# Charrrrrlie/X-as-Supervision

Measured on AMD Instinct MI355X. Metric: images/sec HM36_Multi_SurS1 256px bs32 (full disc+gen training step), higher is better.
Workload: dtype f32 (f16x3 split: every fp32 operand as two fp16 pieces, three products; f32 accumulate); 1 GPU; HM36_Multi_SurS1; batch_per_gpu=32, cameras=4, image=256x256, parallelism=dp1, ranks=1, precision=f16x3, dedupe=False, full=False

## Files before the change

include/xas_hip.h:

```cpp
#ifndef XAS_HIP_H
#define XAS_HIP_H

#include <stddef.h>
#include <stdint.h>

#ifdef __cplusplus
extern "C" {
#endif

const char* xas_last_error(void);
enum {
  XAS_TUNE_WGRAD_SPLIT_XCD = 1,
  XAS_TUNE_PLAIN_KLOOP = 32,
  XAS_TUNE_GLOBAL_LOAD = 64,
  XAS_TUNE_WGRAD_GLOBAL_LOAD = 128,
  XAS_TUNE_WGRAD_ALT_ORDER = 8192,
  XAS_TUNE_WGRAD_PLAIN_KLOOP = 524288,
  XAS_TUNE_SLAB_SHIFT = 15,
  XAS_TUNE_SLAB_MASK = 3,
  XAS_TUNE_SLAB_512 = 32768,
  XAS_TUNE_SLAB_128 = 65536,
  XAS_TUNE_SLAB_64 = 98304,
  XAS_TUNE_COL_REDUCE_LEAN = 262144,
  XAS_TUNE_GENERAL_KERNELS = 1 << 22,
  XAS_TUNE_NO_WIDE_TILES = 1 << 23,
  XAS_TUNE_NO_STEM_WGRAD = 1 << 24,
  XAS_TUNE_STEM_FWD_F32 = 1 << 25,
  XAS_TUNE_NO_X6P = 1 << 26,
  XAS_TUNE_X6P_ANY_K = 1 << 27
};
int xas_set_tuning(int flags);
enum { XAS_PREC_F32 = 0, XAS_PREC_BF16 = 1, XAS_PREC_BF16X6 = 2, XAS_PREC_F16X3 = 3 };
#define XAS_AMAX_SUB 32
#define XAS_AMAX_STRIDE 32
#define XAS_AMAX_SLOT_FLOATS (XAS_AMAX_SUB * XAS_AMAX_STRIDE)
enum { XAS_GRAD_IS_X = 0x100 };
int xas_set_precision(int mode);
int xas_get_precision(void);
int xas_abi_version(void);

#define XAS_HEAD_STATS 16
size_t xas_head_workspace_floats(int B, int K, int D);
int xas_head_softargmax_fwd(const float* logits, int B, int K, int D, int num_hypo, int neighbor,
                            float* kps, int64_t* z_idx, float* depth_prob_map, int groups, float* stats,
                            float* partial, void* stream);
int xas_head_softargmax_from_partials(const float* partial, int B, int K, int D, int nchunk, int num_hypo, int neighbor,
                                      float* kps, int64_t* z_idx, float* depth_prob_map, int groups, float* stats,
                                      void* stream);
int xas_head_softargmax_flip_from_partials(const float* partial, int B, int K, int D, int nchunk, int num_hypo, int neighbor,
                                           const int* perm, float* kps, int64_t* z_idx, float* depth_prob_map, int groups,
                                           void* stream);
int xas_head_softargmax_fwd_flip(const float* logits, int B, int K, int D, int num_hypo, int neighbor, const int* perm,
                                 float* kps, int64_t* z_idx, float* depth_prob_map, int groups, float* partial, void* stream);

int xas_head_softargmax_bwd(const float* logits, const float* stats, const int64_t* z_idx,
                            const float* grad_kps, int B, int K, int D, int num_hypo, int neighbor,
                            float* grad_logits, float* coef, void* stream);
int xas_head_softargmax_bwd_amax(const float* logits, const float* stats, const int64_t* z_idx,
                                 const float* grad_kps, int B, int K, int D, int num_hypo, int neighbor,
                                 float* grad_logits, float* coef, float* amax_out, void* stream);

#define XAS_HEAD_SPREAD 5
size_t xas_head_spread_workspace_floats(int B, int K, int D);
int xas_head_spread(const float* logits, int B, int K, int D, float* spread , float* workspace, void* stream);

#define XAS_GEO_NORM 1
#define XAS_GEO_MONO 2
#define XAS_GEO_PATCH 4
#define XAS_GEO_IMAGE 8
int xas_patch_to_world_fwd(const float* kps, const float* trans_image, const float* k_mat,
                           const float* pelvis, const float* rot_world, const float* trans_world,
                           int B, int Hy, int K, float image_size, float rect_width, int flags,
                           float* world, void* stream);
int xas_patch_to_world_bwd(const float* kps, const float* grad_world, const float* trans_image,
                           const float* k_mat, const float* pelvis, const float* rot_world,
                           const float* trans_world, int B, int Hy, int K, float image_size,
                           float rect_width, int flags, float* grad_kps, void* stream);

#define XAS_GEO_WORLD 16
int xas_world_to_patch_fwd(const float* pts, const float* pre_rot, float pre_scale, int pelvis_origin,
                           const float* trans_image, const float* k_mat, const float* pelvis,
                           const float* rot_world, const float* trans_world, int B, int Hy, int K,
                           float image_size, float rect_width, int flags, float* out, void* stream);
int xas_world_to_patch_bwd(const float* pts, const float* grad_out, const float* pre_rot, float pre_scale,
                           int pelvis_origin, const float* trans_image, const float* k_mat, const float* pelvis,
                           const float* rot_world, const float* trans_world, int B, int Hy, int K,
                           float image_size, float rect_width, int flags, float* grad_pts, float* grad_pre_rot,
                           void* stream);

int xas_lines_nblk(int S);
int xas_draw_lines_max_fwd(const float* kps, long kp_stride_b, long kp_stride_j, int B, int K,
                           const int* parents, const int* children, int L, unsigned fine_mask,
                           float body_width, int S, float* mask, void* stream);
int xas_draw_lines_max_bwd(const float* kps, long kp_stride_b, long kp_stride_j, int B, int K,
                           const int* parents, const int* children, int L, unsigned fine_mask,
                           float body_width, int S, const float* grad_mask, float* partial,
                           float* grad_kps_xy , void* stream);

typedef struct {
  int N, Hi, Wi, Cin;
  int Cout, R, S;
  int stride, pad;
  int Ho, Wo;
  int mode;
  const float* grad_amax;
  const float* x_amax;
} xas_conv_shape;

int xas_conv_weight_planes(const xas_conv_shape* s, int pass);
int xas_conv_kernel_class(const xas_conv_shape* s, int pass);
int xas_f16_weight_overflow(int reset);
int xas_f16_weight_overflow_peek(unsigned* device_out, void* stream);
size_t xas_split_weight_bytes(long rows, long K, int pieces);
// ... 313 lines not shown
```

x-as-supervision_amd/csrc/head.hip:

```cpp
#include "common.h"

namespace xas {

struct HeadGeom {
  int B, K, D, HW, W, C4, G, rec;
  int KT, ntile, C4t;
  int R, rh, rw, wshift;
  int P, nchunk;
};

static int pow2_slots(long C4) {
  int gcd = 1;
  while (gcd < 64 && (C4 % (gcd * 2)) == 0) gcd *= 2;
  return 64 / gcd;
}

static bool pow2_policy(int D, int K) {
  if (!(D >= 4 && D <= 64 && (D & (D - 1)) == 0) || (tune_flags() & XAS_TUNE_GENERAL_KERNELS)) return false;
  if (K <= 0) return true;
  const long C4 = (long)K * (D / 4);
  const int R = pow2_slots(C4);
  return R <= D * D && C4 * R <= 1024;
}

// ... 240 lines not shown
  const float X = a.SX / S, Y = a.SY / S;
  float* st = stats + ((size_t)b * g.K + k) * XAS_HEAD_STATS;
  if (lane == 0) { st[0] = a.M + __logf(S); st[1] = X; st[2] = Y; }
  finalize_tail(g, b, k, pz0, pz1, X, Y, num_hypo, neighbor, kps, z_idx, depth_prob_map, dmap_every, st);
}

__global__ void head_finalize_flip_kernel(const float* __restrict__ partial, HeadGeom g, const int* __restrict__ perm,
                                          int num_hypo, int neighbor, float* __restrict__ kps, int64_t* __restrict__ z_idx,
                                          float* __restrict__ depth_prob_map, int dmap_every) {
  const int b = blockIdx.x / g.K, k = blockIdx.x % g.K;
  const int lane = threadIdx.x;
  const int d0 = lane, d1 = lane + 64;
  const bool live0 = d0 < g.D, live1 = d1 < g.D;
  int k2 = perm[k];
  if ((unsigned)k2 >= (unsigned)g.K) k2 = k;
  const size_t image = (size_t)g.nchunk * g.K * g.rec;
  const ChunkSums a = merge_chunks(partial + b * image + (size_t)k * g.rec, g, d0, d1, live0, live1);
  const ChunkSums m = merge_chunks(partial + ((size_t)(g.B / 2) + b) * image + (size_t)k2 * g.rec, g, d0, d1, live0, live1);
  const float S1 = wave_sum(a.sd0 + a.sd1), S2 = wave_sum(m.sd0 + m.sd1);
  const float pz0 = live0 ? 0.5f * (a.sd0 / S1 + m.sd0 / S2) : 0.f, pz1 = live1 ? 0.5f * (a.sd1 / S1 + m.sd1 / S2) : 0.f;
  const float X = 0.5f * (a.SX / S1 + ((float)(g.W - 1) - m.SX / S2)), Y = 0.5f * (a.SY / S1 + m.SY / S2);
  finalize_tail(g, b, k, pz0, pz1, X, Y, num_hypo, neighbor, kps, z_idx, depth_prob_map, dmap_every, nullptr);
}

__global__ void head_bwd_coef_kernel(const float* __restrict__ stats, const int64_t* __restrict__ z_idx,
                                     const float* __restrict__ grad_kps, HeadGeom g, int num_hypo, int neighbor,
                                     float* __restrict__ coef) {
  const int b = blockIdx.x / g.K, k = blockIdx.x % g.K;
  const int d = threadIdx.x;
  const float* st = stats + ((size_t)b * g.K + k) * XAS_HEAD_STATS;
  const float fD = (float)g.D;
  float gx = 0.f, gy = 0.f, gz = 0.f, c0 = 0.f;
  const int r = neighbor / 2;
  for (int h = 0; h < num_hypo; ++h) {
    const float* gk = grad_kps + (((size_t)b * num_hypo + h) * g.K + k) * 3;
    gx += gk[0];
    gy += gk[1];
    if (neighbor == 0) {
      const float cz = gk[2] * (2.f / fD);
      gz += cz * (float)d;
      c0 -= cz * st[3];
    } else {
      const int idx = (int)z_idx[((size_t)b * g.K + k) * num_hypo + h];
      if (d >= idx - r && d <= idx + r) gz += gk[2] * (2.f / fD) * ((float)d - st[3 + h]) / st[9 + h];
    }
  }
  const float cx = gx * (2.f / fD), cy = gy * (2.f / fD);
  c0 += -cx * st[1] - cy * st[2];
  float* o = coef + ((size_t)b * g.K + k) * (4 + g.D);
  if (d == 0) { o[0] = cx; o[1] = cy; o[2] = c0; o[3] = st[0]; }
  if (d < g.D) o[4 + d] = gz;
}

template <bool POW2>
__global__ void head_bwd_kernel(const float4* __restrict__ logits, const float* __restrict__ coef, HeadGeom g,
                                float4* __restrict__ grad, float* __restrict__ amax_out) {
  __shared__ unsigned s_amax;
  if (threadIdx.x == 0) s_amax = 0u;
  if (amax_out) __syncthreads();
  float amx = 0.f;
  const int KT = POW2 ? g.K : g.KT, C4t = POW2 ? g.C4 : g.C4t;
  const int tid = threadIdx.x;
  const int c4t = tid % C4t, slot = tid / C4t;
  const int kt = c4t / g.G, dq = c4t % g.G;
  const int bz = POW2 ? 0 : blockIdx.z;
  const int k = bz * KT + kt;
  const int b = blockIdx.y, chunk = blockIdx.x;
  const int pix0 = chunk * g.P;
  const int pend = min(g.P, g.HW - pix0);
  if (POW2 || k < g.K) {
    const float* cf = coef + ((size_t)b * g.K + k) * (4 + g.D);
    const float cx = cf[0], cy = cf[1], c0 = cf[2], lse = cf[3];
    const float4 gz = *reinterpret_cast<const float4*>(cf + 4 + 4 * dq);
    const size_t off = ((size_t)b * g.HW + pix0) * g.C4 + (k * g.G + dq);
    PixelWalk<POW2> walk(g, pix0 + slot);
#pragma unroll 4
    for (int p = slot; p < pend; p += g.R) {
      const float4 v = stream_load(logits + off + (size_t)p * g.C4);
      float fh, fw;
      walk.next(g, pix0 + p, &fh, &fw);
      const float lin = cx * fw + cy * fh + c0;
      float4 o;
      o.x = __expf(v.x - lse) * (lin + gz.x);
      o.y = __expf(v.y - lse) * (lin + gz.y);
      o.z = __expf(v.z - lse) * (lin + gz.z);
      o.w = __expf(v.w - lse) * (lin + gz.w);
      amx = amax4(amx, o);
      stream_store(grad + off + (size_t)p * g.C4, o);
    }
  }
  if (amax_out) {
    if (amx > 0.f) atomicMax(&s_amax, __float_as_uint(amx));
    __syncthreads();
    const unsigned sub = (blockIdx.x + (blockIdx.y + bz * gridDim.y) * gridDim.x) % (unsigned)kAmaxSub;
    if (threadIdx.x == 0 && s_amax) atomicMax(reinterpret_cast<unsigned*>(amax_out + sub * kAmaxStride), s_amax);
  }
}

struct SpreadRec { float m, S, uw, uh, Mw, Mh, C; };
constexpr int kSpreadRec = 7;

__device__ __forceinline__ SpreadRec spread_merge(const SpreadRec& a, const SpreadRec& b) {
  SpreadRec r;
  r.m = fmaxf(a.m, b.m);
  const float sa = (a.m == -INFINITY) ? 0.f : __expf(a.m - r.m), sb = (b.m == -INFINITY) ? 0.f : __expf(b.m - r.m);
  const float Sa = a.S * sa, Sb = b.S * sb;
  r.S = Sa + Sb;
  const float f = (r.S == 0.f) ? 0.f : Sb / r.S;
  const float x = Sa * f, dw = b.uw - a.uw, dh = b.uh - a.uh;
  r.uw = a.uw + dw * f;
  r.uh = a.uh + dh * f;
  r.Mw = a.Mw * sa + b.Mw * sb + dw * dw * x;
  r.Mh = a.Mh * sa + b.Mh * sb + dh * dh * x;
  r.C = a.C * sa + b.C * sb + dw * dh * x;
  return r;
}

__device__ __forceinline__ void spread_add(SpreadRec& r, float es, float fw, float fh) {
  const float Sn = r.S + es;
  const float f = (Sn == 0.f) ? 0.f : __fdividef(es, Sn);
  const float x = r.S * f, dw = fw - r.uw, dh = fh - r.uh;
  r.S = Sn;
  r.uw += dw * f;
  r.uh += dh * f;
  r.Mw += dw * dw * x;
  r.Mh += dh * dh * x;
  r.C += dw * dh * x;
}

__device__ __forceinline__ void spread_rescale(SpreadRec& r, float mn) {
  const float sc = __expf(r.m - mn);
  r.m = mn;
  r.S *= sc; r.Mw *= sc; r.Mh *= sc; r.C *= sc;
}

__device__ __forceinline__ SpreadRec spread_read(const float* p) { return {p[0], p[1], p[2], p[3], p[4], p[5], p[6]}; }
__device__ __forceinline__ void spread_write(float* p, const SpreadRec& r) {
  p[0] = r.m; p[1] = r.S; p[2] = r.uw; p[3] = r.uh; p[4] = r.Mw; p[5] = r.Mh; p[6] = r.C;
}

template <bool POW2>
// ... 181 lines not shown
                                                      float* depth_prob_map, int groups, void* stream) {
  XAS_REQUIRE(B > 0 && B <= (1 << 29), "head flip from partials: need 0 < B, got B=%d (the records hold 2B images)", B);
  HeadGeom g;
  if (make_geom(2 * B, K, D, pow2_policy(D, K), &g)) return 1;
  XAS_REQUIRE(partial && perm && kps && depth_prob_map && nchunk >= 1, "head flip from partials: null buffer");
  if (check_modes("head flip from partials", D, num_hypo, neighbor, z_idx, B, groups)) return 1;
  g.nchunk = nchunk;
  return launch_finalize_flip(partial, g, perm, num_hypo, neighbor, kps, z_idx, depth_prob_map, groups, stream);
}

extern "C" int xas_head_softargmax_fwd_flip(const float* logits, int B, int K, int D, int num_hypo, int neighbor, const int* perm,
                                            float* kps, int64_t* z_idx, float* depth_prob_map, int groups, float* partial,
                                            void* stream) {
  XAS_REQUIRE(B > 0 && B <= (1 << 29), "head fwd flip: need 0 < B, got B=%d (the logits hold 2B images)", B);
  const bool pow2 = pow2_policy(D, K);
  HeadGeom g;
  if (make_geom(2 * B, K, D, pow2, &g)) return 1;
  XAS_REQUIRE(logits && perm && kps && depth_prob_map && partial, "head fwd flip: null buffer");
  if (check_modes("head fwd flip", D, num_hypo, neighbor, z_idx, B, groups)) return 1;
  if (launch_partial(logits, partial, g, pow2, "head fwd flip", stream)) return 1;
  return launch_finalize_flip(partial, g, perm, num_hypo, neighbor, kps, z_idx, depth_prob_map, groups, stream);
}

extern "C" size_t xas_head_spread_workspace_floats(int B, int K, int D) {
  HeadGeom g;
  if (make_geom(B, K, D, pow2_policy(D, K), &g)) return 0;
  return (size_t)B * g.nchunk * K * kSpreadRec;
}

extern "C" int xas_head_spread(const float* logits, int B, int K, int D, float* spread, float* workspace, void* stream) {
  const bool pow2 = pow2_policy(D, K);
  HeadGeom g;
  if (make_geom(B, K, D, pow2, &g)) return 1;
  XAS_REQUIRE(logits && spread && workspace, "head spread: null buffer");
  XAS_REQUIRE(((uintptr_t)logits & 15) == 0, "head spread: logits must be 16-byte aligned");
  const size_t lds = spread_lds_bytes(g, pow2);
  XAS_REQUIRE(lds <= 64 * 1024, "head spread: LDS %zu too large", lds);
  XAS_REQUIRE((long)B * K < (1L << 31), "head spread: B=%d K=%d exceed the launch grid", B, K);
  if (check_grid("head spread", g)) return 1;
  hipLaunchKernelGGL(pow2 ? head_spread_partial_kernel<true> : head_spread_partial_kernel<false>, dim3(g.nchunk, g.B, g.ntile),
                     dim3(g.C4t * g.R), lds, as_stream(stream), reinterpret_cast<const float4*>(logits), workspace, g);
  XAS_LAUNCH_CHECK();
  hipLaunchKernelGGL(head_spread_finalize_kernel, dim3(B * K), dim3(64), 0, as_stream(stream), workspace, g, spread);
  XAS_LAUNCH_CHECK();
  return 0;
}

extern "C" int xas_head_softargmax_bwd(const float* logits, const float* stats, const int64_t* z_idx,
                                       const float* grad_kps, int B, int K, int D, int num_hypo, int neighbor,
                                       float* grad_logits, float* coef, void* stream) {
  return xas_head_softargmax_bwd_amax(logits, stats, z_idx, grad_kps, B, K, D, num_hypo, neighbor, grad_logits, coef, nullptr, stream);
}

extern "C" int xas_head_softargmax_bwd_amax(const float* logits, const float* stats, const int64_t* z_idx,
                                            const float* grad_kps, int B, int K, int D, int num_hypo, int neighbor,
                                            float* grad_logits, float* coef, float* amax_out, void* stream) {
  const bool pow2 = pow2_policy(D, K);
  HeadGeom g;
  if (make_geom(B, K, D, pow2, &g)) return 1;
  XAS_REQUIRE(logits && stats && grad_kps && grad_logits && coef, "head bwd: null buffer");
  XAS_REQUIRE(num_hypo >= 1 && num_hypo <= 6, "head bwd: num_hypo %d not in [1,6]", num_hypo);
  XAS_REQUIRE(neighbor == 0 || z_idx != nullptr, "head bwd: z_idx required");
  XAS_REQUIRE((((uintptr_t)logits | (uintptr_t)grad_logits | (uintptr_t)coef) & 15) == 0, "head bwd: 16-byte alignment");
  if (check_grid("head bwd", g)) return 1;
  hipLaunchKernelGGL(head_bwd_coef_kernel, dim3(B * K), dim3(D <= 64 ? 64 : 128), 0, as_stream(stream), stats, z_idx,
                     grad_kps, g, num_hypo, neighbor, coef);
  XAS_LAUNCH_CHECK();
  hipLaunchKernelGGL(pow2 ? head_bwd_kernel<true> : head_bwd_kernel<false>, dim3(g.nchunk, B, g.ntile), dim3(g.C4t * g.R), 0,
                     as_stream(stream), reinterpret_cast<const float4*>(logits), coef, g, reinterpret_cast<float4*>(grad_logits),
                     amax_out);
  XAS_LAUNCH_CHECK();
  return 0;
}
```

x-as-supervision_amd/xas_amd/_lib.py:

```python
import ctypes
import os

import torch

_HERE = os.path.dirname(os.path.abspath(__file__))
LIB_PATH = os.environ.get('XAS_HIP_LIB') or os.path.join(_HERE, 'libxas_hip.so')
_lib = None
ABI_VERSION = 3

_T = {'p': ctypes.c_void_p, 'i': ctypes.c_int, 'l': ctypes.c_long, 'f': ctypes.c_float, 'u': ctypes.c_uint,
      'd': ctypes.c_double, 'z': ctypes.c_size_t}


class ConvShape(ctypes.Structure):
    _fields_ = [(n, ctypes.c_int) for n in ('N', 'Hi', 'Wi', 'Cin', 'Cout', 'R', 'S', 'stride', 'pad', 'Ho', 'Wo', 'mode')] + [
        ('grad_amax', ctypes.c_void_p),
        ('x_amax', ctypes.c_void_p)]


PREC_F32, PREC_BF16, PREC_BF16X6, PREC_F16X3 = 0, 1, 2, 3
PREC_NAMES = {'f32': PREC_F32, 'bf16': PREC_BF16, 'bf16x6': PREC_BF16X6, 'f16x3': PREC_F16X3}

GUARD_FLOATS = 8
GUARD_NORM, GUARD_SCALE, GUARD_SKIP, GUARD_T, GUARD_SKIPPED, GUARD_STEP_SIZE, GUARD_INV_SQRT_BC2, GUARD_NONFINITE = range(8)

TUNE_WGRAD_SPLIT_XCD = 1
TUNE_PLAIN_KLOOP, TUNE_GLOBAL_LOAD, TUNE_WGRAD_GLOBAL_LOAD = 32, 64, 128
TUNE_WGRAD_ALT_ORDER, TUNE_WGRAD_PLAIN_KLOOP = 8192, 524288
TUNE_SLAB_SHIFT, TUNE_SLAB_MASK = 15, 3
TUNE_SLAB_512, TUNE_SLAB_128, TUNE_SLAB_64 = 32768, 65536, 98304
TUNE_COL_REDUCE_LEAN = 262144
TUNE_GENERAL_KERNELS = 1 << 22
TUNE_NO_WIDE_TILES, TUNE_NO_STEM_WGRAD, TUNE_STEM_FWD_F32 = 1 << 23, 1 << 24, 1 << 25
TUNE_NO_X6P, TUNE_X6P_ANY_K = 1 << 26, 1 << 27

PLAN_FIELDS = ('route', 'kernel', 'bm', 'bn', 'pipelined', 'phases', 'pieces', 'patch_width', 'tpb', 'images')
PLAN_ROUTES = (None, 'stem_f16', 'stem_f32', 'thin_vec_to_scalar', 'thin_scalar_to_vec', 'direct', 'mfma')
PLAN_KERNELS = (None, 'igemm_buf', 'igemm', 'igemm_x6', 'igemm_x6t', 'igemm_x6p')


def conv_igemm_plan(shp, pass_, has_bias=False):
    out = (ctypes.c_int * len(PLAN_FIELDS))()
    rc = fn('xas_conv_igemm_plan')(shp, pass_, int(has_bias), ctypes.cast(out, ctypes.c_void_p))
    if rc != 0:
        raise RuntimeError('xas_conv_igemm_plan failed (%d): %s' % (rc, load().xas_last_error().decode()))
    plan = dict(zip(PLAN_FIELDS, out))
    plan['route'], plan['kernel'] = PLAN_ROUTES[plan['route']], PLAN_KERNELS[plan['kernel']]
    return plan


SIGNATURES = {
    'xas_abi_version': ('', 'i'),
    'xas_set_tuning': ('i', 'i'),
    'xas_set_precision': ('i', 'i'),
    'xas_get_precision': ('', 'i'),
    'xas_conv_weight_planes': ('si', 'i'),
    'xas_conv_kernel_class': ('si', 'i'),
    'xas_f16_weight_overflow': ('i', 'i'),
    'xas_f16_weight_overflow_peek': ('pp', 'i'),
    'xas_split_weight_bytes': ('lli', 'z'),
    'xas_split_weight': ('ppllip', 'i'),
    'xas_prepare_weights': ('pilp', 'i'),
    'xas_head_workspace_floats': ('iii', 'z'),
    'xas_head_softargmax_fwd': ('piiiiipppippp', 'i'),
    'xas_head_softargmax_bwd': ('ppppiiiiippp', 'i'),
    'xas_head_softargmax_bwd_amax': ('ppppiiiiipppp', 'i'),
    'xas_patch_to_world_fwd': ('ppppppiiiffipp', 'i'),
    'xas_patch_to_world_bwd': ('pppppppiiiffipp', 'i'),
    'xas_world_to_patch_fwd': ('ppfipppppiiiffipp', 'i'),
    'xas_world_to_patch_bwd': ('pppfipppppiiiffippp', 'i'),
    'xas_lines_nblk': ('i', 'i'),
    'xas_draw_lines_max_fwd': ('plliippiufipp', 'i'),
    'xas_draw_lines_max_bwd': ('plliippiufipppp', 'i'),
    'xas_conv_fwd': ('ppppsp', 'i'),
    'xas_conv_fwd_head_chunks': ('sii', 'i'),
    'xas_conv_fwd_head': ('ppppsiipp', 'i'),
    'xas_head_softargmax_from_partials': ('piiiiiipppipp', 'i'),
    'xas_head_softargmax_flip_from_partials': ('piiiiiippppip', 'i'),
    'xas_head_softargmax_fwd_flip': ('piiiiippppipp', 'i'),
    'xas_head_spread_workspace_floats': ('iii', 'z'),
    'xas_head_spread': ('piiippp', 'i'),
    'xas_conv_fwd_bnstats_workspace_floats': ('si', 'z'),
    'xas_conv_fwd_bnstats': ('pppsippplppppfp', 'i'),
    'xas_conv_dgrad_bn_bwd_workspace_floats': ('si', 'z'),
    'xas_conv_dgrad_bn_bwd': ('ppspppppfidppppppp', 'i'),
    'xas_conv_dgrad': ('pppsp', 'i'),
    'xas_conv_dgrad_acc': ('pppsp', 'i'),
    'xas_conv_dgrad_acc_masked': ('pppsppp', 'i'),
    'xas_conv_igemm_plan': ('siip', 'i'),
    'xas_conv_wgrad_workspace_floats': ('s', 'z'),
    'xas_conv_wgrad': ('ppppsp', 'i'),
    'xas_conv_wgrad_oihw': ('ppppsp', 'i'),
    'xas_conv_wgrad_acc': ('ppppsp', 'i'),
    'xas_pack_weight': ('ppiiiiip', 'i'),
    'xas_unpack_weight': ('ppiiiiip', 'i'),
    'xas_bn_workspace_floats': ('lii', 'z'),
    'xas_bn_stats': ('pliipplppppflp', 'i'),
    'xas_bn_stats_from_partials': ('pliilppplppppfp', 'i'),
    'xas_bn_bwd_sums_from_partials': ('pliippppp', 'i'),
    'xas_bn_sync_merge': ('piiilppppfp', 'i'),
    'xas_col_sum': ('plippp', 'i'),
    'xas_col_sum_acc': ('plippp', 'i'),
    'xas_bn_apply': ('ppppppfiliippp', 'i'),
    'xas_bn_apply_amax': ('ppppppfiliipppp', 'i'),
    'xas_abs_max': ('plpp', 'i'),
    'xas_bn_update_running': ('ppppfliip', 'i'),
    'xas_bn_bwd_reduce': ('pppppppfiliipppppp', 'i'),
    'xas_bn_bwd_apply': ('ppppppppfiliidpppp', 'i'),
    'xas_bn_bwd_apply_amax': ('ppppppppfiliidppppp', 'i'),
    'xas_bn_apply_dual_amax': ('pppppf' 'pppppf' 'lii' 'pppp', 'i'),
    'xas_bn_bwd_reduce_dual': ('ppppppf' 'ppf' 'lii' 'ppp' 'pppp' 'p', 'i'),
    'xas_bn_bwd_apply_dual_amax': ('pppp' 'ppppf' 'ppppf' 'liidd' 'pppp' 'p', 'i'),
    'xas_maxpool3x3s2_fwd': ('piiiippp', 'i'),
    'xas_maxpool3x3s2_bwd': ('ppiiiipp', 'i'),
    'xas_upsample2x_fwd': ('piiiipp', 'i'),
    'xas_upsample2x_bwd': ('piiiipp', 'i'),
    'xas_sigmoid_fwd': ('plpp', 'i'),
    'xas_sigmoid_bwd': ('pplpp', 'i'),
    'xas_nchw_to_nhwc': ('piiiipp', 'i'),
# ... 66 lines not shown
        raise RuntimeError('libxas_hip.so is missing (%s): run `python __graft_entry__.py` to build the HIP '
                           'library; the MI355X path has no CPU fallback' % LIB_PATH)
    lib = ctypes.CDLL(LIB_PATH)
    lib.xas_abi_version.restype = ctypes.c_int
    lib.xas_abi_version.argtypes = []
    if lib.xas_abi_version() != ABI_VERSION:
        raise RuntimeError('%s speaks ABI version %d, this binding expects %d (include/xas_hip.h): rebuild it with '
                           '`python __graft_entry__.py`' % (LIB_PATH, lib.xas_abi_version(), ABI_VERSION))
    lib.xas_last_error.restype = ctypes.c_char_p
    lib.xas_last_error.argtypes = []
    _lib = lib
    mode = os.environ.get('XAS_PRECISION', '')
    if mode != '':
        lib.xas_set_precision.argtypes = [ctypes.c_int]
        lib.xas_set_precision.restype = ctypes.c_int
        if lib.xas_set_precision(int(mode)) != 0:
            raise RuntimeError('XAS_PRECISION=%s: %s' % (mode, lib.xas_last_error().decode()))
    global PREC_DEFAULT
    lib.xas_get_precision.restype = ctypes.c_int
    PREC_DEFAULT = int(lib.xas_get_precision())
    return lib


PREC_DEFAULT = None


_bound = {}


def fn(name):
    f = _bound.get(name)
    if f is None:
        args, ret = SIGNATURES[name]
        f = getattr(load(), name)
        f.argtypes = [ctypes.POINTER(ConvShape) if c == 's' else _T[c] for c in args]
        f.restype = _T[ret]
        _bound[name] = f
    return f


def ptr(t):
    if t is None:
        return None
    if not t.is_cuda:
        raise RuntimeError('xas_amd ops run on the GPU only (got a %s tensor); there is no CPU fallback' % t.device)
    return t.data_ptr()


def stream():
    return torch.cuda.current_stream().cuda_stream


profiler = None


def call(name, *args):
    if profiler is not None and name in profiler.names:
        return profiler.timed_call(name, args)
    rc = fn(name)(*args, stream())
    if rc != 0:
        raise RuntimeError('%s failed (%d): %s' % (name, rc, load().xas_last_error().decode()))


def query(name, *args):
    return fn(name)(*args)
```

x-as-supervision_amd/xas_amd/ops_head.py:

```python
import torch

from . import _lib
from ._lib import call, ptr, query

HEAD_STATS = 16
peak_probe = None
GEO_NORM, GEO_MONO, GEO_PATCH = 1, 2, 4
GEO_IMAGE, GEO_WORLD = 8, 16


def _nhwc_storage(logits):
    if logits.dim() != 4:
        raise RuntimeError('logits must be [B, K*D, H, W]')
    if not logits.is_contiguous(memory_format=torch.channels_last):
        logits = logits.contiguous(memory_format=torch.channels_last)
    return logits


def check_patch_size(x, depth_dim, who):
    if x.dim() != 4 or x.shape[-1] != x.shape[-2] or x.shape[-1] != 4 * depth_dim:
        raise RuntimeError('%s(depth_dim=%d) takes square input patches of side 4 * depth_dim = %d, got input %s: build the '
                           'detector with depth_dim = patch size / 4 (a multiple of 4, at most 128: patches up to 512)'
                           % (who, depth_dim, 4 * depth_dim, tuple(x.shape)))


class _SoftArgmax(torch.autograd.Function):
    @staticmethod
    def forward(ctx, logits, num_kp, num_hypo, neighbor, groups):
        from . import ops_nn
        logits_in = logits
        logits_tail = _nhwc_storage(logits)
        logits = ops_nn._full(logits_tail)
        B, C, H, W = logits.shape
        D = C // num_kp
        if not (C == num_kp * D and D == H == W):
            raise RuntimeError('soft-argmax head needs a heat-map cube D == H == W with D a multiple of 4 in [4,128] '
                               '(got C=%d K=%d H=%d W=%d)' % (C, num_kp, H, W))
        dev = logits.device
        kps = torch.empty(B, num_hypo, num_kp, 3, device=dev, dtype=torch.float32)
        z_idx = torch.empty(B, num_kp, num_hypo, device=dev, dtype=torch.int64)
        dmap = torch.empty(groups, num_kp, D, device=dev, dtype=torch.float32)
        stats = torch.empty(B, num_kp, HEAD_STATS, device=dev, dtype=torch.float32)
        pre = getattr(logits_in, '_xas_head', None)
        if pre is not None and pre[2] == logits_in._version and pre[0].shape[0] == B and pre[0].shape[2] == num_kp:
            ops_nn.head_stats['fused'] += 1
            call('xas_head_softargmax_from_partials', ptr(pre[0]), B, num_kp, D, pre[1], num_hypo, neighbor, ptr(kps), ptr(z_idx),
                 ptr(dmap), groups, ptr(stats))
        else:
            ops_nn.head_stats['separate'] += 1
            ws = torch.empty(query('xas_head_workspace_floats', B, num_kp, D), device=dev, dtype=torch.float32)
            call('xas_head_softargmax_fwd', ptr(logits), B, num_kp, D, num_hypo, neighbor, ptr(kps), ptr(z_idx),
                 ptr(dmap), groups, ptr(stats), ptr(ws))
        if peak_probe is not None:
            peak_probe(z_idx.clone())
        s = B - logits_tail.shape[0]
        kps_prefix = kps[:s] if s else kps[:0]
        kps, z_idx_all = (kps[s:], z_idx) if s else (kps, z_idx)
        ctx.save_for_backward(logits_tail, stats[s:] if s else stats, z_idx[s:] if s else z_idx)
        ctx.cfg = (num_kp, D, num_hypo, neighbor)
        ctx.mark_non_differentiable(z_idx_all, dmap, kps_prefix)
        return kps, dmap, z_idx_all, kps_prefix

    @staticmethod
    def backward(ctx, g_kps, _g_dmap, _g_idx, _g_prefix=None):
        logits, stats, z_idx = ctx.saved_tensors
        K, D, Hy, nb = ctx.cfg
        B = logits.shape[0]
        g_kps = g_kps.contiguous()
        grad = torch.empty_like(logits)
        coef = torch.empty(B * K * (4 + D), device=logits.device, dtype=torch.float32)
        from . import ops_nn
        slot = ops_nn.grad_amax_slot(logits.device)
        call('xas_head_softargmax_bwd_amax', ptr(logits), ptr(stats), ptr(z_idx), ptr(g_kps), B, K, D, Hy, nb,
             ptr(grad), ptr(coef), ptr(slot))
        if slot is not None:
            ops_nn.tag_grad_amax(grad, slot)
        return grad, None, None, None, None


def softargmax_multi(logits, num_kp, num_hypo, neighbor_size, groups=1):
    kps, dmap, idx, prefix = _SoftArgmax.apply(logits, num_kp, num_hypo, neighbor_size, groups)
    _last_prefix[0] = prefix
    return kps, (dmap[0] if groups == 1 else dmap), idx


_last_prefix = [None]


def softargmax_single(logits, num_kp, groups=1):
    kps, dmap, _, prefix = _SoftArgmax.apply(logits, num_kp, 1, 0, groups)
    _last_prefix[0] = prefix
    return kps, (dmap[0] if groups == 1 else dmap)


def flip_perm(flip_pairs, num_kp, device):
    perm = list(range(num_kp))
    for pair in flip_pairs:
        a, b = (int(v) for v in pair)
        if not (0 <= a < num_kp and 0 <= b < num_kp) or a == b:
            raise RuntimeError('flip pair (%d, %d) does not name two of the %d joints' % (a, b, num_kp))
        if perm[a] != a or perm[b] != b:
            raise RuntimeError('flip pair (%d, %d): a joint has two partners' % (a, b))
        perm[a], perm[b] = b, a
    t = torch.tensor(perm, dtype=torch.int32, device=device)
    t._xas_perm_k = num_kp
    return t


def softargmax_flip(heatmap_2b, num_kp, num_hypo, neighbor_size, perm, groups=1):
    from . import ops_nn
    if torch.is_grad_enabled() and heatmap_2b.requires_grad:
        raise RuntimeError('softargmax_flip is an inference path without a backward: call it under torch.no_grad()')
    if ops_nn._prefix[0]:
        raise RuntimeError('softargmax_flip does not run inside a prefix pass')
    logits = _nhwc_storage(heatmap_2b)
    B2, C, H, W = logits.shape
    D = C // num_kp
    if not (C == num_kp * D and D == H == W):
        raise RuntimeError('soft-argmax head needs a heat-map cube D == H == W with D a multiple of 4 in [4,128] '
                           '(got C=%d K=%d H=%d W=%d)' % (C, num_kp, H, W))
    if B2 < 2 or B2 % 2:
        raise RuntimeError('softargmax_flip takes the logits of B images followed by their B mirrors, got %d images' % B2)
    B = B2 // 2
    dev = logits.device
    if not isinstance(perm, torch.Tensor):
        perm = torch.as_tensor(perm)
    if getattr(perm, '_xas_perm_k', None) != num_kp:
        host = perm.detach().cpu().reshape(-1).tolist()
        if len(host) != num_kp or any(int(v) != v or not 0 <= v < num_kp for v in host):
            raise RuntimeError('softargmax_flip: perm must hold %d joint indices in [0, %d), got %s' % (num_kp, num_kp, host))
        perm = perm.to(device=dev, dtype=torch.int32).contiguous()
        perm._xas_perm_k = num_kp
    if perm.device != dev or perm.dtype != torch.int32 or not perm.is_contiguous():
        raise RuntimeError('softargmax_flip: perm must be a contiguous int32 tensor on %s' % dev)
    kps = torch.empty(B, num_hypo, num_kp, 3, device=dev, dtype=torch.float32)
    z_idx = torch.zeros(B, num_kp, num_hypo, device=dev, dtype=torch.int64)
    dmap = torch.empty(groups, num_kp, D, device=dev, dtype=torch.float32)
    pre = getattr(heatmap_2b, '_xas_head', None)
    if pre is not None and pre[2] == heatmap_2b._version and pre[0].shape[0] == B2 and pre[0].shape[2] == num_kp:
        ops_nn.head_stats['fused'] += 1
        call('xas_head_softargmax_flip_from_partials', ptr(pre[0]), B, num_kp, D, pre[1], num_hypo, neighbor_size, ptr(perm),
             ptr(kps), ptr(z_idx), ptr(dmap), groups)
    else:
# ... 191 lines not shown
```

x-as-supervision_amd/xas_amd/ops_nn.py:

```python
import os

import torch
import torch.distributed as dist

from . import _lib
from . import streams
from ._lib import ConvShape, call, ptr, query

CL = torch.channels_last
_weights_epoch = [0]

_groups = [1]

_prefix = [0, 0]


class bn_groups:
    def __init__(self, groups, prefix_groups=0, images_per_group=0):
        self.groups = int(groups)
        self.prefix = [int(prefix_groups) * int(images_per_group), int(prefix_groups)]
        if self.prefix[1] and not (0 < self.prefix[1] < self.groups and images_per_group > 0):
            raise RuntimeError('bn_groups: the no-grad prefix must be a proper, non-empty subset of the groups')

    def __enter__(self):
        self.prev, _groups[0] = _groups[0], self.groups
        self.prev_prefix = list(_prefix)
        _prefix[0], _prefix[1] = self.prefix
        return self

    def __exit__(self, *exc):
        _groups[0] = self.prev
        _prefix[0], _prefix[1] = self.prev_prefix
        if not _prefix[0]:
            _prefix_storages.clear()


_prefix_storages = set()


def mark_prefix_buffer(buf):
    _prefix_storages.add(buf.untyped_storage().data_ptr())


def _full(x):
    s = _prefix[0]
    if not s or x is None:
        return x
    per = x.stride(0)
    off = x.storage_offset() - s * per
    if (x.dim() != 4 or not x.is_contiguous(memory_format=CL) or off < 0
            or (x.storage_offset() + x.numel()) * 4 > x.untyped_storage().nbytes()
            or x.untyped_storage().data_ptr() not in _prefix_storages):
        raise RuntimeError('prefix pass: an activation arrived without its %d prefix images in front of it' % s)
# ... 328 lines not shown
        box = getattr(w, '_xas_epoch', _weights_epoch)
        key = (w.data_ptr(), w._version, box[0])
        if key != self.key:
            self.key, self.packed = key, {}

    def get(self, w, transposed, shp=None, planes=None):
        self._fresh(w)
        if planes is None:
            planes = query('xas_conv_weight_planes', shp, int(transposed)) if shp is not None else 0
        k = (transposed, planes)
        if k in self.packed:
            return self.packed[k]
        if (transposed, 0) not in self.packed:
            co, ci, r, s = w.shape
            if not transposed and r == 1 and s == 1 and w.is_contiguous() and w.data_ptr() % 16 == 0:
                self.packed[(transposed, 0)] = w.detach().view(-1)
            else:
                p = torch.empty(w.numel(), device=w.device, dtype=torch.float32)
                call('xas_pack_weight', ptr(w.detach().contiguous()), ptr(p), co, ci, r, s, int(transposed))
                self.packed[(transposed, 0)] = p
        if planes:
            src = self.packed[(transposed, 0)]
            rows = w.shape[1] if transposed else w.shape[0]
            kk = src.numel() // rows
            sp = torch.empty(query('xas_split_weight_bytes', rows, kk, planes), device=w.device, dtype=torch.uint8)
            call('xas_split_weight', ptr(src), ptr(sp), rows, kk, planes)
            self.packed[k] = sp
        return self.packed[k]


def _col_sum(t2d_ptr_tensor, M, C):
    out = torch.empty(C, device=t2d_ptr_tensor.device, dtype=torch.float32)
    ws = torch.empty(query('xas_bn_workspace_floats', M, C, 1), device=out.device, dtype=torch.float32)
    call('xas_col_sum', ptr(t2d_ptr_tensor), M, C, ptr(out), ptr(ws))
    return out


def _bias_grad(dy, M, C):
    if C % 4 == 0:
        return _col_sum(dy, M, C)
    return dy.reshape(M, C).sum(0)


def _wgrad(x, dy, shp, w_shape, transposed=False):
    co, ci, r, s = shp.Cout, shp.Cin, shp.R, shp.S
    ws = torch.empty(max(1, query('xas_conv_wgrad_workspace_floats', shp)), device=x.device, dtype=torch.float32)
    dw = torch.empty(w_shape, device=x.device, dtype=torch.float32)
    call('xas_conv_wgrad_oihw', ptr(x), ptr(dy), ptr(dw), ptr(ws), shp)
    return dw


HEAD_IN_EPILOGUE = os.environ.get('XAS_HEAD_IN_EPILOGUE', '1') == '1'
head_stats = {'fused': 0, 'separate': 0}


class _Conv2d(torch.autograd.Function):
    @staticmethod
    def forward(ctx, x, weight, bias, stride, pad, cache, head_kd=None):
        x = to_cl(x)
        n, ci, hi, wi = x.shape
        co, ci2, r, s = weight.shape
        if ci != ci2:
            raise RuntimeError('conv2d: input has %d channels, weight expects %d' % (ci, ci2))
        ho, wo = (hi + 2 * pad - r) // stride + 1, (wi + 2 * pad - s) // stride + 1
        shp, x_slot = with_act_amax(_shape(n, hi, wi, ci, co, r, s, stride, pad, ho, wo), x)
        xf = _full(x)
        yf = empty_cl(xf.shape[0], co, ho, wo, x)
        shp_f = _with_n(shp, xf.shape[0])
        chunks = query('xas_conv_fwd_head_chunks', shp_f, head_kd[0], head_kd[1]) if (head_kd and HEAD_IN_EPILOGUE and x.is_cuda) else 0
        if chunks:
            rec = torch.empty(xf.shape[0], chunks, head_kd[0], 3 + head_kd[1], device=x.device, dtype=torch.float32)
            call('xas_conv_fwd_head', ptr(xf), ptr(cache.get(weight, 0, shp_f)), ptr(bias), ptr(yf), shp_f, head_kd[0], head_kd[1], ptr(rec))
        else:
            call('xas_conv_fwd', ptr(xf), ptr(cache.get(weight, 0, shp_f)), ptr(bias), ptr(yf), shp_f)
        y = _tail(yf)
        if chunks:
            y._xas_head = (rec, chunks, y._version)
        ctx.save_for_backward(x, weight, *([bias] if bias is not None else []))
        ctx.shp, ctx.cache, ctx.has_bias, ctx.x_slot = shp, cache, bias is not None, x_slot
        if ctx.needs_input_grad[1]:
            note_use(weight)
        if bias is not None and ctx.needs_input_grad[2]:
            note_use(bias)
        return y

    @staticmethod
    def backward(ctx, dy):
        x, weight, *rest = ctx.saved_tensors
        shp = with_grad_amax(ctx.shp, dy, ctx.x_slot)
        dy = to_cl(dy)
        dx = dw = db = None
        if ctx.needs_input_grad[0]:
            dx = torch.empty_like(x)
            call('xas_conv_dgrad', ptr(dy), ptr(ctx.cache.get(weight, 1, shp)), ptr(dx), shp)
        if ctx.needs_input_grad[1] and not _wgrad_into_grad(x, dy, shp, weight):
            dw = _wgrad(x, dy, shp, weight.shape)
        if ctx.has_bias and ctx.needs_input_grad[2]:
            M = shp.N * shp.Ho * shp.Wo
            if not _bias_into_grad(dy, M, shp.Cout, rest[0]):
                db = _bias_grad(dy, M, shp.Cout)
        return dx, dw, db, None, None, None, None


def conv2d(x, weight, bias, stride, pad, cache, head_kd=None):
    return _Conv2d.apply(x, weight, bias, stride, pad, cache, head_kd)


def _conv_forward(x, weight, stride, pad, cache):
    n, ci, hi, wi = x.shape
    co, ci2, r, s = weight.shape
    if ci != ci2:
        raise RuntimeError('conv2d: input has %d channels, weight expects %d' % (ci, ci2))
    ho, wo = (hi + 2 * pad - r) // stride + 1, (wi + 2 * pad - s) // stride + 1
    shp, _ = with_act_amax(_shape(n, hi, wi, ci, co, r, s, stride, pad, ho, wo), x)
    xf = _full(x)
    yf = empty_cl(xf.shape[0], co, ho, wo, x)
    shp_f = _with_n(shp, xf.shape[0])
    call('xas_conv_fwd', ptr(xf), ptr(cache.get(weight, 0, shp_f)), None, ptr(yf), shp_f)
    return _tail(yf), shp


FUSE_CONV_STATS = os.environ.get('XAS_CONV_STATS', '1') == '1'


def _conv_bn_forward(x, conv, bn, residual, group, stats_only=False, proj=None):
    weight = conv.weight
    if not (FUSE_CONV_STATS and bn.training):
        y, shp = _conv_forward(x, weight, conv.stride, conv.padding, conv._cache)
        out, sv, cf = _bn_forward(y, bn.weight, bn.bias, bn.running_mean, bn.running_var, residual, bn.training,
                                  bn.momentum, bn.eps, bn.act, group, stats_only=stats_only, proj=proj)
        return out, sv, cf, shp
    n, ci, hi, wi = x.shape
    co, ci2, r, s = weight.shape
    if ci != ci2:
        raise RuntimeError('conv2d: input has %d channels, weight expects %d' % (ci, ci2))
    stride, pad = conv.stride, conv.padding
    ho, wo = (hi + 2 * pad - r) // stride + 1, (wi + 2 * pad - s) // stride + 1
    shp, _ = with_act_amax(_shape(n, hi, wi, ci, co, r, s, stride, pad, ho, wo), x)
    xf = _full(x)
    shp_f = _with_n(shp, xf.shape[0])
    yf = empty_cl(xf.shape[0], co, ho, wo, x)
    y = _tail(yf)
    wp = conv._cache.get(weight, 0, shp_f)
    G = _groups[0]
    pivot = None

    def stats(mean_p, var_p, out_stride, count_p, rm_p, rv_p, momentum):
        ws = torch.empty(query('xas_conv_fwd_bnstats_workspace_floats', shp_f, G), device=x.device, dtype=torch.float32)
        call('xas_conv_fwd_bnstats', ptr(xf), ptr(wp), ptr(yf), shp_f, G, ptr(pivot), mean_p, var_p, out_stride, count_p,
             ptr(ws), rm_p, rv_p, float(momentum))

    out, sv, cf = _bn_forward(y, bn.weight, bn.bias, bn.running_mean, bn.running_var, residual, True, bn.momentum,
# ... 735 lines not shown
```

x-as-supervision_amd/xas_amd/prof.py:

```python
import torch

from . import _lib

CONV_ENTRIES = ('xas_conv_fwd', 'xas_conv_fwd_head', 'xas_conv_fwd_bnstats', 'xas_conv_dgrad', 'xas_conv_dgrad_acc', 'xas_conv_dgrad_acc_masked', 'xas_conv_wgrad',
                'xas_conv_wgrad_oihw', 'xas_conv_wgrad_acc')


BN_ENTRIES = ('xas_bn_stats', 'xas_bn_apply', 'xas_bn_apply_amax', 'xas_bn_bwd_reduce', 'xas_bn_bwd_apply', 'xas_bn_bwd_apply_amax',
              'xas_bn_apply_dual_amax', 'xas_bn_bwd_reduce_dual', 'xas_bn_bwd_apply_dual_amax')


def bn_bytes(name, a):
    if name == 'xas_bn_stats':
        return 4.0 * a[1] * a[2]
    if name in ('xas_bn_apply', 'xas_bn_apply_amax'):
        t = 4.0 * a[8] * a[9]
        return t * (2 + (1 if a[5] else 0)) + (t / 16 if a[12] else 0.0)
    if name == 'xas_bn_bwd_reduce':
        t = 4.0 * a[9] * a[10]
        return t * (1 + (1 if a[0] else 0) + (1 if a[1] else 0)) + (t / 16 if a[16] else 0.0)
    if name == 'xas_bn_apply_dual_amax':
        t = 4.0 * a[12] * a[13]
        return t * 3 + t / 16
    if name == 'xas_bn_bwd_reduce_dual':
# ... 6 lines not shown
    return t * (2 + (1 if a[0] else 0) + (1 if a[1] else 0) + (1 if a[15] else 0)) + (t / 16 if a[16] else 0.0)


def conv_flops(shape):
    return 2.0 * shape.N * shape.Ho * shape.Wo * shape.Cout * shape.R * shape.S * shape.Cin


def conv_bytes(shape):
    return 4.0 * (shape.N * shape.Hi * shape.Wi * shape.Cin + shape.Cout * shape.R * shape.S * shape.Cin
                  + shape.N * shape.Ho * shape.Wo * shape.Cout)


class KernelTimer:
    def __init__(self, names=CONV_ENTRIES):
        self.names = set(names)
        self.records = []
        self.bytes_total = 0.0

    def __enter__(self):
        _lib.profiler = self
        return self

    def __exit__(self, *exc):
        _lib.profiler = None

    def timed_call(self, name, args):
        shape = next((a for a in args if isinstance(a, _lib.ConvShape)), None)
        a, b = torch.cuda.Event(enable_timing=True), torch.cuda.Event(enable_timing=True)
        a.record()
        rc = _lib.fn(name)(*args, _lib.stream())
        b.record()
        if rc != 0:
            raise RuntimeError('%s failed (%d): %s' % (name, rc, _lib.load().xas_last_error().decode()))
        mfma = 0
        if shape is not None:
            kind = 0 if name in ('xas_conv_fwd', 'xas_conv_fwd_head', 'xas_conv_fwd_bnstats') else (
                1 if name in ('xas_conv_dgrad', 'xas_conv_dgrad_acc', 'xas_conv_dgrad_acc_masked', 'xas_conv_dgrad_bn_bwd') else 2)
            mfma = _lib.query('xas_conv_kernel_class', shape, kind)
        sig = None
        if shape is not None:
            sig = (shape.N, shape.Hi, shape.Wi, shape.Cin, shape.Cout, shape.R, shape.stride)
        work = conv_flops(shape) if shape is not None else 0.0
        if name == 'xas_head_softargmax_fwd':
            B, K, D = args[1], args[2], args[3]
            work, sig = 4.0 * B * K * D * D * D, (B, K, D)
        elif name == 'xas_head_softargmax_from_partials':
            B, K, D, nch = args[1], args[2], args[3], args[4]
            work, sig = 4.0 * B * nch * K * (3 + D), (B, K, D)
        elif name in BN_ENTRIES:
            work, sig = bn_bytes(name, args), None
        elif name in ('xas_head_softargmax_bwd', 'xas_head_softargmax_bwd_amax'):
            B, K, D = args[4], args[5], args[6]
            work, sig = 8.0 * B * K * D * D * D, (B, K, D)
        self.records.append((name, a, b, work, mfma, sig))
        self.bytes_total += conv_bytes(shape) if (shape is not None and mfma) else 0.0

    CLASS = {0: ':direct', 1: ':f32', 2: ':bf16', 3: ':bf16x6', 4: ':f16x3'}

    def summary(self):
        out = {}
        for name, a, b, fl, mfma, _sig in self.records:
            key = name + (self.CLASS[mfma] if name.startswith('xas_conv') else '')
            d = out.setdefault(key, {'launches': 0, 'ms': 0.0, 'flops': 0.0})
            d['launches'] += 1
            d['ms'] += a.elapsed_time(b)
            d['flops'] += fl
        return out

    def by_shape(self):
        agg = {}
        for name, a, b, fl, mfma, sig in self.records:
            d = agg.setdefault((name, sig), [0, 0.0, 0.0])
            d[0] += 1
            d[1] += a.elapsed_time(b)
            d[2] += fl
        rows = [(k[0], k[1], v[0], v[1], (v[2] / (v[1] * 1e-3) / 1e12) if v[1] > 0 else 0.0) for k, v in agg.items()]
        return sorted(rows, key=lambda r: -r[3])
```

Measured before the change: 2128 images/s.

## Fuse final-conv bias gradient column sums into soft-argmax head backward

The head backward kernel gains a variant that accumulates per-chunk column sums of the gradient it writes, reduces them through LDS, and then runs a small column-sum pass into the bias-gradient buffer. The final convolution's backward picks up these sums when the arriving gradient is the same tensor the head wrote, instead of re-reading the whole logits gradient to compute the bias gradient. This removes one full read pass over a large activation-gradient tensor. In exchange it adds LDS traffic, a block sync, a workspace allocation and an extra small reduction launch, plus autograd plumbing that links the head op to the conv node.

```diff
diff --git a/include/xas_hip.h b/include/xas_hip.h
--- a/include/xas_hip.h
+++ b/include/xas_hip.h
@@ -59,6 +59,11 @@
 int xas_head_softargmax_bwd_amax(const float* logits, const float* stats, const int64_t* z_idx,
                                  const float* grad_kps, int B, int K, int D, int num_hypo, int neighbor,
                                  float* grad_logits, float* coef, float* amax_out, void* stream);
+size_t xas_head_bwd_colsum_workspace_floats(int B, int K, int D);
+int xas_head_softargmax_bwd_colsum(const float* logits, const float* stats, const int64_t* z_idx,
+                                   const float* grad_kps, int B, int K, int D, int num_hypo, int neighbor,
+                                   float* grad_logits, float* coef, float* amax_out, float* workspace, float* colsum_acc,
+                                   void* stream);
 
 #define XAS_HEAD_SPREAD 5
 size_t xas_head_spread_workspace_floats(int B, int K, int D);
diff --git a/x-as-supervision_amd/csrc/head.hip b/x-as-supervision_amd/csrc/head.hip
--- a/x-as-supervision_amd/csrc/head.hip
+++ b/x-as-supervision_amd/csrc/head.hip
@@ -316,9 +316,16 @@
   if (d < g.D) o[4 + d] = gz;
 }
 
-template <bool POW2>
+__device__ __forceinline__ void sum4_stored(float4& a, const float4& o) {
+#pragma clang fp contract(off)
+  a.x = a.x + o.x; a.y = a.y + o.y; a.z = a.z + o.z; a.w = a.w + o.w;
+}
+
+template <bool POW2, bool SUMS = false>
 __global__ void head_bwd_kernel(const float4* __restrict__ logits, const float* __restrict__ coef, HeadGeom g,
-                                float4* __restrict__ grad, float* __restrict__ amax_out) {
+                                float4* __restrict__ grad, float* __restrict__ amax_out, float4* __restrict__ colsum) {
+  extern __shared__ float4 s_sum[];
+  float4 acc = make_float4(0.f, 0.f, 0.f, 0.f);
   __shared__ unsigned s_amax;
   if (threadIdx.x == 0) s_amax = 0u;
   if (amax_out) __syncthreads();
@@ -349,8 +356,21 @@
       o.y = __expf(v.y - lse) * (lin + gz.y);
       o.z = __expf(v.z - lse) * (lin + gz.z);
       o.w = __expf(v.w - lse) * (lin + gz.w);
+      if constexpr (SUMS) sum4_stored(acc, o);
       amx = amax4(amx, o);
       stream_store(grad + off + (size_t)p * g.C4, o);
+    }
+  }
+  if constexpr (SUMS) {
+    s_sum[tid] = acc;
+    __syncthreads();
+    if (slot == 0 && (POW2 || k < g.K)) {
+      float4 t = s_sum[c4t];
+      for (int s = 1; s < g.R; ++s) {
+        const float4 u = s_sum[s * C4t + c4t];
+        t.x += u.x; t.y += u.y; t.z += u.z; t.w += u.w;
+      }
+      colsum[((size_t)b * g.nchunk + chunk) * g.C4 + (k * g.G + dq)] = t;
     }
   }
   if (amax_out) {
@@ -638,9 +658,9 @@
   return xas_head_softargmax_bwd_amax(logits, stats, z_idx, grad_kps, B, K, D, num_hypo, neighbor, grad_logits, coef, nullptr, stream);
 }
 
-extern "C" int xas_head_softargmax_bwd_amax(const float* logits, const float* stats, const int64_t* z_idx,
-                                            const float* grad_kps, int B, int K, int D, int num_hypo, int neighbor,
-                                            float* grad_logits, float* coef, float* amax_out, void* stream) {
+static int head_bwd_launch(const float* logits, const float* stats, const int64_t* z_idx, const float* grad_kps, int B, int K, int D,
+                           int num_hypo, int neighbor, float* grad_logits, float* coef, float* amax_out, float* colsum_ws,
+                           float* colsum_acc, void* stream) {
   const bool pow2 = pow2_policy(D, K);
   HeadGeom g;
   if (make_geom(B, K, D, pow2, &g)) return 1;
@@ -652,9 +672,42 @@
   hipLaunchKernelGGL(head_bwd_coef_kernel, dim3(B * K), dim3(D <= 64 ? 64 : 128), 0, as_stream(stream), stats, z_idx,
                      grad_kps, g, num_hypo, neighbor, coef);
   XAS_LAUNCH_CHECK();
-  hipLaunchKernelGGL(pow2 ? head_bwd_kernel<true> : head_bwd_kernel<false>, dim3(g.nchunk, B, g.ntile), dim3(g.C4t * g.R), 0,
+  const dim3 grid(g.nchunk, B, g.ntile), block(g.C4t * g.R);
+  if (!colsum_acc) {
+    hipLaunchKernelGGL(pow2 ? head_bwd_kernel<true> : head_bwd_kernel<false>, grid, block, 0, as_stream(stream),
+                       reinterpret_cast<const float4*>(logits), coef, g, reinterpret_cast<float4*>(grad_logits), amax_out,
+                       static_cast<float4*>(nullptr));
+    XAS_LAUNCH_CHECK();
+    return 0;
+  }
+  const long rows = (long)B * g.nchunk;
+  hipLaunchKernelGGL((pow2 ? head_bwd_kernel<true, true> : head_bwd_kernel<false, true>), grid, block, block.x * sizeof(float4),
                      as_stream(stream), reinterpret_cast<const float4*>(logits), coef, g, reinterpret_cast<float4*>(grad_logits),
-                     amax_out);
+                     amax_out, reinterpret_cast<float4*>(colsum_ws));
   XAS_LAUNCH_CHECK();
-  return 0;
-}
+  return xas_col_sum_acc(colsum_ws, rows, K * D, colsum_acc, colsum_ws + (size_t)rows * K * D, stream);
+}
+
+extern "C" int xas_head_softargmax_bwd_amax(const float* logits, const float* stats, const int64_t* z_idx,
+                                            const float* grad_kps, int B, int K, int D, int num_hypo, int neighbor,
+                                            float* grad_logits, float* coef, float* amax_out, void* stream) {
+  return head_bwd_launch(logits, stats, z_idx, grad_kps, B, K, D, num_hypo, neighbor, grad_logits, coef, amax_out, nullptr, nullptr,
+                         stream);
+}
+
+extern "C" size_t xas_head_bwd_colsum_workspace_floats(int B, int K, int D) {
+  HeadGeom g;
+  if (make_geom(B, K, D, pow2_policy(D, K), &g)) return 0;
+  const long rows = (long)B * g.nchunk;
+  return (size_t)rows * K * D + xas_bn_workspace_floats(rows, K * D, 1);
+}
+
+extern "C" int xas_head_softargmax_bwd_colsum(const float* logits, const float* stats, const int64_t* z_idx,
+                                              const float* grad_kps, int B, int K, int D, int num_hypo, int neighbor,
+                                              float* grad_logits, float* coef, float* amax_out, float* workspace,
+                                              float* colsum_acc, void* stream) {
+  XAS_REQUIRE(workspace && colsum_acc && (((uintptr_t)workspace | (uintptr_t)colsum_acc) & 15) == 0,
+              "head bwd colsum: null / misaligned workspace or destination");
+  return head_bwd_launch(logits, stats, z_idx, grad_kps, B, K, D, num_hypo, neighbor, grad_logits, coef, amax_out, workspace,
+                         colsum_acc, stream);
+}
diff --git a/x-as-supervision_amd/xas_amd/_lib.py b/x-as-supervision_amd/xas_amd/_lib.py
--- a/x-as-supervision_amd/xas_amd/_lib.py
+++ b/x-as-supervision_amd/xas_amd/_lib.py
@@ -65,6 +65,8 @@
     'xas_head_softargmax_fwd': ('piiiiipppippp', 'i'),
     'xas_head_softargmax_bwd': ('ppppiiiiippp', 'i'),
     'xas_head_softargmax_bwd_amax': ('ppppiiiiipppp', 'i'),
+    'xas_head_bwd_colsum_workspace_floats': ('iii', 'z'),
+    'xas_head_softargmax_bwd_colsum': ('ppppiiiiipppppp', 'i'),
     'xas_patch_to_world_fwd': ('ppppppiiiffipp', 'i'),
     'xas_patch_to_world_bwd': ('pppppppiiiffipp', 'i'),
     'xas_world_to_patch_fwd': ('ppfipppppiiiffipp', 'i'),
@@ -237,10 +239,11 @@
 
 
 profiler = None
+PROFILE_AS = {'xas_head_softargmax_bwd_colsum': 'xas_head_softargmax_bwd_amax'}
 
 
 def call(name, *args):
-    if profiler is not None and name in profiler.names:
+    if profiler is not None and PROFILE_AS.get(name, name) in profiler.names:
         return profiler.timed_call(name, args)
     rc = fn(name)(*args, stream())
     if rc != 0:
diff --git a/x-as-supervision_amd/xas_amd/ops_head.py b/x-as-supervision_amd/xas_amd/ops_head.py
--- a/x-as-supervision_amd/xas_amd/ops_head.py
+++ b/x-as-supervision_amd/xas_amd/ops_head.py
@@ -26,8 +26,9 @@
 
 class _SoftArgmax(torch.autograd.Function):
     @staticmethod
-    def forward(ctx, logits, num_kp, num_hypo, neighbor, groups):
+    def forward(ctx, logits, num_kp, num_hypo, neighbor, groups, conv_node=None):
         from . import ops_nn
+        ctx.conv_node = conv_node
         logits_in = logits
         logits_tail = _nhwc_storage(logits)
         logits = ops_nn._full(logits_tail)
@@ -71,15 +72,25 @@
         coef = torch.empty(B * K * (4 + D), device=logits.device, dtype=torch.float32)
         from . import ops_nn
         slot = ops_nn.grad_amax_slot(logits.device)
-        call('xas_head_softargmax_bwd_amax', ptr(logits), ptr(stats), ptr(z_idx), ptr(g_kps), B, K, D, Hy, nb,
-             ptr(grad), ptr(coef), ptr(slot))
+        node = ctx.conv_node
+        if node is not None:
+            sums = torch.zeros(K * D, device=logits.device, dtype=torch.float32)
+            ws = torch.empty(query('xas_head_bwd_colsum_workspace_floats', B, K, D), device=logits.device, dtype=torch.float32)
+            call('xas_head_softargmax_bwd_colsum', ptr(logits), ptr(stats), ptr(z_idx), ptr(g_kps), B, K, D, Hy, nb,
+                 ptr(grad), ptr(coef), ptr(slot), ptr(ws), ptr(sums))
+        else:
+            call('xas_head_softargmax_bwd_amax', ptr(logits), ptr(stats), ptr(z_idx), ptr(g_kps), B, K, D, Hy, nb,
+                 ptr(grad), ptr(coef), ptr(slot))
         if slot is not None:
             ops_nn.tag_grad_amax(grad, slot)
-        return grad, None, None, None, None
+        if node is not None:
+            node.head_bias = (grad, grad._version, sums)
+        return grad, None, None, None, None, None
 
 
 def softargmax_multi(logits, num_kp, num_hypo, neighbor_size, groups=1):
-    kps, dmap, idx, prefix = _SoftArgmax.apply(logits, num_kp, num_hypo, neighbor_size, groups)
+    from . import ops_nn
+    kps, dmap, idx, prefix = _SoftArgmax.apply(logits, num_kp, num_hypo, neighbor_size, groups, ops_nn.head_conv_node(logits))
     _last_prefix[0] = prefix
     return kps, (dmap[0] if groups == 1 else dmap), idx
 
@@ -88,7 +99,8 @@
 
 
 def softargmax_single(logits, num_kp, groups=1):
-    kps, dmap, _, prefix = _SoftArgmax.apply(logits, num_kp, 1, 0, groups)
+    from . import ops_nn
+    kps, dmap, _, prefix = _SoftArgmax.apply(logits, num_kp, 1, 0, groups, ops_nn.head_conv_node(logits))
     _last_prefix[0] = prefix
     return kps, (dmap[0] if groups == 1 else dmap)
 
diff --git a/x-as-supervision_amd/xas_amd/ops_nn.py b/x-as-supervision_amd/xas_amd/ops_nn.py
--- a/x-as-supervision_amd/xas_amd/ops_nn.py
+++ b/x-as-supervision_amd/xas_amd/ops_nn.py
@@ -1,4 +1,5 @@
 import os
+import warnings
 
 import torch
 import torch.distributed as dist
@@ -433,6 +434,35 @@
 
 HEAD_IN_EPILOGUE = os.environ.get('XAS_HEAD_IN_EPILOGUE', '1') == '1'
 head_stats = {'fused': 0, 'separate': 0}
+
+
+HEAD_BIAS_FUSE = os.environ.get('XAS_HEAD_BIAS_FUSE', '1') == '1'
+head_bias_stats = {'fused': 0, 'refused': 0}
+
+
+def head_conv_node(logits):
+    if not (HEAD_BIAS_FUSE and torch.is_grad_enabled() and logits.is_cuda and logits.requires_grad):
+        return None
+    node = logits.grad_fn
+    if not isinstance(node, _Conv2d._backward_cls) or not getattr(node, 'has_bias', False) or not node.needs_input_grad[2]:
+        return None
+    return node
+
+
+def _bias_from_head(ctx, dy, bias):
+    left = ctx.__dict__.pop('head_bias', None)
+    if left is None:
+        return None
+    grad, version, sums = left
+    if (dy.data_ptr() == grad.data_ptr() and dy._version == version and dy.shape == grad.shape and dy.stride() == grad.stride()
+            and sums.numel() == bias.numel()):
+        head_bias_stats['fused'] += 1
+        return sums
+    head_bias_stats['refused'] += 1
+    if head_bias_stats['refused'] == 1:
+        warnings.warn('final convolution: the gradient that arrived is not the one the soft-argmax head wrote (another consumer '
+                      'of the logits, or a copy in between): its bias gradient is summed in a pass of its own')
+    return None
 
 
 class _Conv2d(torch.autograd.Function):
@@ -469,6 +499,7 @@
     def backward(ctx, dy):
         x, weight, *rest = ctx.saved_tensors
         shp = with_grad_amax(ctx.shp, dy, ctx.x_slot)
+        head_sums = _bias_from_head(ctx, dy, rest[0]) if ctx.has_bias else None
         dy = to_cl(dy)
         dx = dw = db = None
         if ctx.needs_input_grad[0]:
@@ -478,7 +509,10 @@
             dw = _wgrad(x, dy, shp, weight.shape)
         if ctx.has_bias and ctx.needs_input_grad[2]:
             M = shp.N * shp.Ho * shp.Wo
-            if not _bias_into_grad(dy, M, shp.Cout, rest[0]):
+            if head_sums is not None:
+                if not _bias_into_grad(head_sums, 1, shp.Cout, rest[0]):
+                    db = head_sums
+            elif not _bias_into_grad(dy, M, shp.Cout, rest[0]):
                 db = _bias_grad(dy, M, shp.Cout)
         return dx, dw, db, None, None, None, None
 
diff --git a/x-as-supervision_amd/xas_amd/prof.py b/x-as-supervision_amd/xas_amd/prof.py
--- a/x-as-supervision_amd/xas_amd/prof.py
+++ b/x-as-supervision_amd/xas_amd/prof.py
@@ -82,6 +82,10 @@
         elif name in ('xas_head_softargmax_bwd', 'xas_head_softargmax_bwd_amax'):
             B, K, D = args[4], args[5], args[6]
             work, sig = 8.0 * B * K * D * D * D, (B, K, D)
+        elif name == 'xas_head_softargmax_bwd_colsum':
+            B, K, D = args[4], args[5], args[6]
+            work, sig = 8.0 * B * K * D * D * D + 8.0 * _lib.query('xas_head_bwd_colsum_workspace_floats', B, K, D), (B, K, D)
+        name = _lib.PROFILE_AS.get(name, name)
         self.records.append((name, a, b, work, mfma, sig))
         self.bytes_total += conv_bytes(shape) if (shape is not None and mfma) else 0.0
 
```

Result: no change. 2142 images/s (median of 6 runs) (+0.6%).
